# yabebalFantaye/MCEvidence

Hardware: AMD Instinct MI355X
Metric: knn_queries_per_sec (higher is better)
Workload: dtype f16 filter + f64 refine (exact f64 results)

## Files before the change

mcevidence_amd/csrc/f16_filter.hpp:

```cpp
#pragma once
#include <math.h>
#include <stdint.h>
#if defined(__HIPCC__)
#include <hip/hip_runtime.h>
#endif

#include "sym_types.hpp"

namespace mce {

#if defined(__HIPCC__)
#define MCE_HDI __host__ __device__ __forceinline__
#else
#define MCE_HDI inline
#endif

enum { HP_RMAX = 0, HP_SCALE = 1, HP_EY = 2, HP_YHATMAX = 3, HP_RHO = 4, HP_STAT_CHUNKS = 5, HP_STAT_TILES = 6, HP_COUNT = 16 };

constexpr int kHWaves = 8;
constexpr int kHThreads = kHWaves * 64;
constexpr int kHRelBits = 26;
constexpr int kHSymRowBits = kHRelBits - 1;

MCE_HDI float f16_round_up(double g)
{
#if defined(__HIP_DEVICE_COMPILE__)
    return __double2float_ru(g);
#else
    float f = (float)g;
    if ((double)f < g) f = nextafterf(f, __builtin_huge_valf());
    return f;
#endif
}
struct F16GateTerms { double a, c, eps; };
MCE_HDI double f16_gate_a(double ex, double ey, int KST) { return (ex + ey) * (1.0 + 1e-9) + 2.0 * sqrt(16.0 * KST) * 0x1p-14; }
MCE_HDI F16GateTerms f16_gate_terms(double ex, double xn, double ey, double ymax, double rho, int KST, bool live = true)
{
    const double r = sqrt(xn) + ymax;
    const double a = f16_gate_a(ex, ey, KST);
    const double eps = (32.0 * KST) * 0x1p-24 * r * r * (1.0 + 0x1p-9) + rho + 1e-30;
    return {a, live ? eps - xn : -__builtin_huge_val(), eps};
}
MCE_HDI double f16_reach2(double thr, double s2, double a)
{
    const double rr = sqrt(thr * s2) * (1.0 + 1e-12) + a;
    return rr * rr * (1.0 + 1e-12);
}
MCE_HDI float f16_gate_finite(double thr, double s2, double a, double c) { return f16_round_up(f16_reach2(thr, s2, a) + c); }
MCE_HDI float f16_gate(double thr, double s2, double a, double c)
{
    if (!(c > -__builtin_huge_val())) return -__builtin_huge_valf();
    if (!(thr < __builtin_huge_val())) return __builtin_huge_valf();
    return f16_gate_finite(thr, s2, a, c);
}
MCE_HDI double f16_row_const(double ymax) { return 0x1p-22 * (ymax * ymax + 1.0); }
MCE_HDI float f16_row_round(double g, double rowc) { return f16_round_up(g * (1.0 + 0x1p-22) + rowc + 1e-30); }
MCE_HDI float f16_row_gate(double thr, double s2, double a, double rowc)
{
    if (!(thr < __builtin_huge_val())) return __builtin_huge_valf();
    return f16_row_round(f16_reach2(thr, s2, a), rowc);
}
template <class P>
MCE_HDI float f16_row_gate_of(double thr, double ex, P params, int KST)
{
    if (!(thr < __builtin_huge_val())) return __builtin_huge_valf();
    const double s2 = params[HP_SCALE] * params[HP_SCALE];
    const double g = f16_reach2(thr, s2, f16_gate_a(ex, params[HP_EY], KST));
    return f16_row_round(g, f16_row_const(params[HP_YHATMAX]));
}
MCE_HDI double f16_seed_bound(double a_up, double xn, double eps, double a, double s2)
{
    const double dd = sqrt(fmax(a_up + xn + eps, 0.0)) * (1.0 + 1e-12) + a;
    return dd * dd * (1.0 + 1e-12) / s2 * (1.0 + 1e-12);
}

template <int N, class D, class I>
MCE_HD inline void list_insert(D&& own_d, I&& own_i, double d2, int j)
{
    const double INF = __builtin_huge_val();
    bool c_hi = (d2 < own_d[N - 1]) || (d2 == own_d[N - 1] && j < own_i[N - 1] && d2 < INF);
#pragma unroll
    for (int k = N - 1; k >= 1; --k) {
        const bool c_lo = (d2 < own_d[k - 1]) || (d2 == own_d[k - 1] && j < own_i[k - 1] && d2 < INF);
        own_d[k] = c_lo ? own_d[k - 1] : (c_hi ? d2 : own_d[k]);
        own_i[k] = c_lo ? own_i[k - 1] : (c_hi ? j : own_i[k]);
        c_hi = c_lo;
    }
    own_d[0] = c_hi ? d2 : own_d[0];
    own_i[0] = c_hi ? j : own_i[0];
}

#if defined(__HIPCC__)
typedef _Float16 v8h __attribute__((ext_vector_type(8)));
typedef float v16f __attribute__((ext_vector_type(16)));

__device__ __forceinline__ float min3f(float a, float b, float c)
{
    float r;
    asm("v_min3_f32 %0, %1, %2, %3" : "=v"(r) : "v"(a), "v"(b), "v"(c));
    return r;
}
__device__ __forceinline__ void f16_min16_halves(const v16f& c, float (&l1)[5], float& m0, float& m3)
{
    l1[0] = min3f(c[0], c[1], c[2]);
    l1[1] = min3f(c[3], c[4], c[5]);
    l1[2] = min3f(c[6], c[7], c[8]);
    l1[3] = min3f(c[9], c[10], c[11]);
    l1[4] = min3f(c[12], c[13], c[14]);
    m0 = min3f(l1[0], l1[1], l1[2]);
    m3 = min3f(l1[3], l1[4], c[15]);
}
__device__ __forceinline__ float f16_min16(const v16f& c, float (&l1)[5])
{
    float m0, m3;
    f16_min16_halves(c, l1, m0, m3);
    return min3f(m0, m3, m3);
}
__device__ __forceinline__ float f16_min16(const v16f& c, float (&l1)[5], float run)
{
    float m0, m3;
    f16_min16_halves(c, l1, m0, m3);
    return min3f(run, m0, m3);
}

template <int KCAP, class PS, class PT, class PR, class PF, class RG>
__device__ __forceinline__ bool sym_slot_insert(PS slots, PT thr, PR rrow, PF rtile, int ksel, int row, double d2, RG row_gate)
{
    const auto sl = slots + (int64_t)row * KCAP;
    for (;;) {
        double vmax = -1.0, v2 = -1.0;
        int imax = 0;
#pragma unroll
        for (int k = 0; k < KCAP; ++k) {
            if (k < ksel) {
                const double v = __longlong_as_double((long long)__hip_atomic_load(sl + k, __ATOMIC_RELAXED, __HIP_MEMORY_SCOPE_AGENT));
                if (v > vmax) { v2 = vmax; vmax = v; imax = k; }
                else if (v > v2) v2 = v;
            }
        }
        if (d2 > vmax) return false;
        if (d2 == vmax) return true;
        unsigned long long expect = (unsigned long long)__double_as_longlong(vmax);
        if (__hip_atomic_compare_exchange_strong(sl + imax, &expect, (unsigned long long)__double_as_longlong(d2), __ATOMIC_RELAXED,
                                                 __ATOMIC_RELAXED, __HIP_MEMORY_SCOPE_AGENT)) {
            const double nk = fmax(v2, d2);
            if (nk < __builtin_huge_val()) {
                const unsigned long long nb = (unsigned long long)__double_as_longlong(nk);
                const unsigned long long ob = __hip_atomic_fetch_min(thr + row, nb, __ATOMIC_RELAXED, __HIP_MEMORY_SCOPE_AGENT);
                if (nb < ob) {
                    const unsigned rb = __float_as_uint(row_gate(nk, row));
                    const unsigned orb = __hip_atomic_fetch_min(rrow + row, rb, __ATOMIC_RELAXED, __HIP_MEMORY_SCOPE_AGENT);
                    if (rb < orb) {
                        const auto rt = rrow + (int64_t)(row >> 5) * 32;
                        unsigned m = 0;
                        for (int k = 0; k < 32; ++k) {
                            const unsigned v = __hip_atomic_load(rt + k, __ATOMIC_RELAXED, __HIP_MEMORY_SCOPE_AGENT);
                            m = v > m ? v : m;
                        }
                        __hip_atomic_store(rtile + (row >> 5), __uint_as_float(m), __ATOMIC_RELAXED, __HIP_MEMORY_SCOPE_AGENT);
                    }
                }
            }
            return true;
        }
    }
}

template <bool ROWFLAG>
__device__ __forceinline__ unsigned f16_event(const v16f& c, const float (&l1)[5], const unsigned lanew, const float g, const bool rowflag, const int jb0,
                                              const unsigned todo, const int qlimit, int* const wq, int& qcount)
{
    const unsigned wbase = (lanew + (unsigned)jb0) | (ROWFLAG && rowflag ? (1u << kHSymRowBits) : 0u);
    unsigned rem = 0;
#define MCE_HIT(R_, P_, S_)                                                                                               \
    if ((S_) != 0 && (todo & (1u << (R_)))) {                                                                             \
        if (qcount > qlimit) rem |= 1u << (R_);                                                                           \
        else {                                                                                                            \
            if (P_) wq[__builtin_amdgcn_mbcnt_hi((unsigned)((S_) >> 32), __builtin_amdgcn_mbcnt_lo((unsigned)(S_), (unsigned)qcount))] = \
                        (int)(wbase + (unsigned)(((R_) & 3) + 8 * ((R_) >> 2)));                                          \
            qcount += __builtin_popcountll(S_);                                                                           \
        }                                                                                                                 \
    }
#define MCE_TRIPLE(I_, U_)                                                                                                \
    if ((U_) != 0) {                                                                                                      \
        const bool p0 = c[3 * (I_) + 0] <= g, p1 = c[3 * (I_) + 1] <= g, p2 = c[3 * (I_) + 2] <= g;                     \
        const unsigned long long s0 = __ballot(p0), s1 = __ballot(p1), s2 = __ballot(p2);                                \
        MCE_HIT(3 * (I_) + 0, p0, s0)                                                                                     \
        MCE_HIT(3 * (I_) + 1, p1, s1)                                                                                     \
        MCE_HIT(3 * (I_) + 2, p2, s2)                                                                                     \
    }
    const bool q0 = l1[0] <= g, q1 = l1[1] <= g, q2 = l1[2] <= g, q3 = l1[3] <= g, q4 = l1[4] <= g, p15 = c[15] <= g;
    const unsigned long long u0 = __ballot(q0), u1 = __ballot(q1), u2 = __ballot(q2), u3 = __ballot(q3), u4 = __ballot(q4), s15 = __ballot(p15);
    MCE_TRIPLE(0, u0) MCE_TRIPLE(1, u1) MCE_TRIPLE(2, u2) MCE_TRIPLE(3, u3) MCE_TRIPLE(4, u4)
    MCE_HIT(15, p15, s15)
#undef MCE_TRIPLE
#undef MCE_HIT
    return rem;
}

template <int VPT, class P>
__device__ __forceinline__ void f16_stage_chunk(P src, char* dst, int tid, int wave)
{
#pragma unroll
    for (int i = 0; i < VPT; ++i) {
        const int e = tid + i * kHThreads;
        __builtin_amdgcn_global_load_lds(
            (const __attribute__((address_space(1))) void*)(src + (size_t)e * 16),
            (__attribute__((address_space(3))) void*)(dst + (size_t)(wave * 64 + i * kHThreads) * 16),
            16, 0, 0);
    }
}
template <int KST>
__device__ __forceinline__ void f16_load_a(const char* lp, v8h (&a)[KST])
{
#pragma unroll
    for (int ks = 0; ks < KST; ++ks) a[ks] = *reinterpret_cast<const v8h*>(lp + ks * 1024);
}

#endif

}
```

mcevidence_amd/csrc/knn_panel.hpp:

```cpp
#pragma once
#include "knn_f16.hpp"

namespace mce {

struct PanelArgs {
    const _Float16* Yh;
    const _Float16* Xh;
    const double* qinfo;
    const double* params;
    const double* X;
    const double* Y;
    const int* rperm;
    double* part_d;
    int* part_i;
    int64_t nq, nr, nq_pad, self_offset;
    int D, ksel, self_exclude, spin_limit;
    int debug;
    SymParams sym;
    PanelGeom geom;
    const PanelUnit* units = nullptr;
    const double* lo_d = nullptr;
    const int* lo_i = nullptr;
};

#ifndef MCE_PANEL_STATS
#define MCE_PANEL_STATS 0
#endif
#ifndef MCE_PANEL_NPASS
#define MCE_PANEL_NPASS 3
#endif
#ifndef MCE_PANEL_STAGE_KB
#define MCE_PANEL_STAGE_KB MCE_H_STAGE_KB
#endif
#ifndef MCE_PANEL_QUEUE
#define MCE_PANEL_QUEUE MCE_H_QUEUE
#endif
#ifndef MCE_PANEL_TRIGGER
#define MCE_PANEL_TRIGGER 192
#endif
#ifndef MCE_PANEL_ABL
#define MCE_PANEL_ABL 0
#endif

__host__ __device__ constexpr int panel_chunk_tiles(int KST) { return MCE_PANEL_STAGE_KB / KST / 2 * 2; }
constexpr int kPanelQueue = MCE_PANEL_QUEUE;
__host__ __device__ constexpr size_t panel_lds_bytes(int KST)
{
    return (size_t)2 * panel_chunk_tiles(KST) * KST * 1024
           + (size_t)kHWaves * kPanelQueue * 16
           + (size_t)kHWaves * kHQT * 32 * 4 + 128
           + (size_t)kHWaves * kHQT * 32 * 4
           + (size_t)kHWaves * panel_chunk_tiles(KST) * kHQT * 4;
}

template <class T> __device__ __forceinline__ const __attribute__((address_space(1))) T* gptr(const T* p)
{
    return (const __attribute__((address_space(1))) T*)p;
}
template <class T> __device__ __forceinline__ __attribute__((address_space(1))) T* gptr_w(T* p)
{
    return (__attribute__((address_space(1))) T*)p;
}

__device__ __forceinline__ float vmaxf(float a, float b)
{
    float r;
    asm("v_max_f32 %0, %1, %2" : "=v"(r) : "v"(a), "v"(b));
    return r;
}

template <int KST, int KCAP, bool LOWER = false>
__global__ __launch_bounds__(kHThreads, 2) void knn_panel_kernel(PanelArgs args_by_value)
{
    static_assert(kHQT == 2 && kHNL == 1, "8 waves x 2 query tiles, one list per owner lane");
    constexpr int QT = 2;
    constexpr int QPW = 64;
    constexpr int QPB = kHWaves * QPW;
    constexpr int TPB = QPB / 32;
    constexpr int CT = panel_chunk_tiles(KST);
    constexpr int CHUNK_BYTES = CT * KST * 1024;
    constexpr int VPT = CHUNK_BYTES / 16 / kHThreads;
    static_assert(CHUNK_BYTES % (16 * kHThreads) == 0 && CT % 2 == 0, "chunk geometry");
    constexpr int QN = kPanelQueue;
    (void)args_by_value;
    typedef const __attribute__((address_space(4))) PanelArgs* ArgsPtr;
    const ArgsPtr ap0 = (ArgsPtr)__builtin_amdgcn_kernarg_segment_ptr();
#define MCE_ARGS() ([&]() __attribute__((always_inline)) { ArgsPtr p_ = ap0; asm volatile("" : "+s"(p_)); return p_; }())

    extern __shared__ __attribute__((aligned(16))) char lds_raw[];
    char* const stage0 = lds_raw;
    double* const qd2_all = reinterpret_cast<double*>(lds_raw + 2 * CHUNK_BYTES);
    int* const qpk_all = reinterpret_cast<int*>(qd2_all + kHWaves * QN);
    int* const qnx_all = qpk_all + kHWaves * QN;
    int* const head_all = qnx_all + kHWaves * QN;
    volatile int* const wvote = head_all + kHWaves * QPW;
    float* const sthr_all = reinterpret_cast<float*>(head_all + kHWaves * QPW + 32);
    int* const redo_all = reinterpret_cast<int*>(sthr_all + kHWaves * QPW);

    const int tid = threadIdx.x;
    const int lane = tid & 63;
    const int wave = __builtin_amdgcn_readfirstlane(tid >> 6);
    double* const wqd = qd2_all + wave * QN;
    int* const wq = qpk_all + wave * QN;
    int* const wnx = qnx_all + wave * QN;
    int* const whead = head_all + wave * QPW;
    float* const sthr = sthr_all + wave * QPW;
    int* const wredo = redo_all + wave * (CT * QT);
    const double INF = __builtin_huge_val();

#if MCE_PANEL_STATS
    const long long t_kernel0 = clock64();
    long long st_drains = 0, st_enq = 0, st_events = 0, st_redo = 0, st_tD = 0, st_tE = 0, st_tPro = 0, st_tA = 0, st_tR = 0, st_tB = 0;
#endif

    int sym_p, qblk, t_lo, t_hi, useq, sym_on, qb_lo;
    {
        const ArgsPtr a = MCE_ARGS();
        if (a->units) {
            const auto u = (const __attribute__((address_space(1))) PanelUnit*)a->units + blockIdx.x;
            qblk = __builtin_amdgcn_readfirstlane(u->qblk);
            t_lo = __builtin_amdgcn_readfirstlane(u->t_lo);
            t_hi = __builtin_amdgcn_readfirstlane(u->t_hi);
            useq = __builtin_amdgcn_readfirstlane(u->useq);
            sym_p = 0;
            sym_on = a->geom.sym_on;
            qb_lo = a->geom.qb_lo;
        } else {
            PanelGeom g;
            g.qb_lo = a->geom.qb_lo; g.qb_hi = a->geom.qb_hi; g.tpb = a->geom.tpb; g.tpp = a->geom.tpp;
            g.ct = a->geom.ct; g.ntiles = a->geom.ntiles; g.sym_on = a->geom.sym_on;
            panel_unit_decode((int)blockIdx.x, g, sym_p, qblk);
            panel_unit_tiles(sym_p, qblk, g, t_lo, t_hi);
            useq = panel_unit_seq(sym_p, qblk, g);
            sym_on = g.sym_on;
            qb_lo = g.qb_lo;
        }
    }
    auto chain_of = [&](int& chain, int64_t& list_off) __attribute__((always_inline)) {
        const ArgsPtr a = MCE_ARGS();
        chain = qblk;
        list_off = 0;
        if (a->units) {
            const auto u = (const __attribute__((address_space(1))) PanelUnit*)a->units + blockIdx.x;
            chain = __builtin_amdgcn_readfirstlane(u->chain);
            list_off = (int64_t)__builtin_amdgcn_readfirstlane(u->list_set) * KCAP * a->nq_pad;
        }
    };
    const int64_t qwave0 = (int64_t)qblk * QPB + wave * QPW;

    whead[lane] = -1;
    if (tid < 3) wvote[tid] = 0;

    double own_d[KCAP];
    int own_i[KCAP];
#pragma unroll
    for (int k = 0; k < KCAP; ++k) { own_d[k] = INF; own_i[k] = -1; }
    double seed_thr = INF;

    {
        const ArgsPtr a = MCE_ARGS();
        if (useq > 0) {
            int chain;
            int64_t list_off;
            chain_of(chain, list_off);
            int spins = 0;
            const int limit = ((a->debug & 16) && useq == 1 && (wave & 1)) ? -1 : a->spin_limit;
            bool ok = true;
            const auto done = gptr(a->sym.done);
            while (spins > limit || __hip_atomic_load(done + chain, __ATOMIC_RELAXED, __HIP_MEMORY_SCOPE_AGENT) < useq) {
                if (++spins > limit) { ok = false; break; }
                __builtin_amdgcn_s_sleep(32);
            }
            __builtin_amdgcn_fence(__ATOMIC_ACQUIRE, "agent");
            if (ok && gptr(a->sym.bucket_flag)[qblk] != 0) ok = false;
            if (ok) {
                const int64_t q = qwave0 + lane;
                const int64_t np = a->nq_pad;
                const auto pd = gptr(a->part_d) + list_off;
                const auto pi = gptr(a->part_i) + list_off;
#pragma unroll
                for (int k = 0; k < KCAP; ++k) {
                    own_d[k] = pd[(int64_t)k * np + q];
                    own_i[k] = pi[(int64_t)k * np + q];
                }
            } else if (lane == 0) {
                gptr_w(a->sym.bucket_flag)[qblk] = 1;
            }
        }
    }

    v8h b[QT][KST];
    float G[QT], cR[QT];
    unsigned lanew[QT];
    const int k_last = MCE_ARGS()->ksel - 1;
    {
        const ArgsPtr a = MCE_ARGS();
        const auto Xh = gptr(a->Xh);
#pragma unroll
        for (int qt = 0; qt < QT; ++qt) {
            const int64_t q = qwave0 + qt * 32 + (lane & 31);
#pragma unroll
            for (int ks = 0; ks < KST; ++ks)
                b[qt][ks] = *(const __attribute__((address_space(1))) v8h*)(Xh + q * (int64_t)(16 * KST) + 16 * ks + 8 * (lane >> 5));
            lanew[qt] = ((unsigned)(qt * 32 + (lane & 31)) << kHRelBits) | (unsigned)(4 * (lane >> 5));
            cR[qt] = -__builtin_huge_valf();
            G[qt] = -__builtin_huge_valf();
        }
    }
    double gq_a[QT], gq_c[QT], own_a = 0.0, s2c, rowc;
    {
        const ArgsPtr a = MCE_ARGS();
        const auto params = gptr(a->params);
        const auto qinfo = gptr(a->qinfo);
        const double p_scale = params[HP_SCALE], p_ey = params[HP_EY], p_ym = params[HP_YHATMAX], p_rho = params[HP_RHO];
        s2c = p_scale * p_scale;
        rowc = f16_row_const(p_ym);
#pragma unroll
        for (int qt = 0; qt < QT; ++qt) {
            const int64_t q = qwave0 + qt * 32 + (lane & 31);
            gq_a[qt] = 0.0;
            gq_c[qt] = -INF;
            if (q < a->nq && MCE_PANEL_ABL != 1) {
                const F16GateTerms t = f16_gate_terms(qinfo[2 * q], qinfo[2 * q + 1], p_ey, p_ym, p_rho, KST);
                gq_a[qt] = t.a;
                gq_c[qt] = t.c;
            }
        }
        {
            const int64_t q = qwave0 + lane;
            if (q < a->nq) own_a = f16_gate_a(qinfo[2 * q], p_ey, KST);
        }
    }
    auto gate_of = [&](double thr, int qt) __attribute__((always_inline)) -> float { return f16_gate(thr, s2c, gq_a[qt], gq_c[qt]); };
    auto own_row_gate = [&](double thr) __attribute__((always_inline)) -> float { return f16_row_gate(thr, s2c, own_a, rowc); };
    {
        const ArgsPtr a = MCE_ARGS();
        const int64_t q = qwave0 + lane;
        double t0 = INF;
        if (sym_on) t0 = __longlong_as_double((long long)__hip_atomic_load(gptr(a->sym.thr) + q, __ATOMIC_RELAXED, __HIP_MEMORY_SCOPE_AGENT));
        else if (a->sym.thr) t0 = __longlong_as_double((long long)gptr(a->sym.thr)[q]);
        seed_thr = t0;
        double tl = own_d[KCAP - 1];
#pragma unroll
        for (int k = 0; k < KCAP - 1; ++k) tl = (k == k_last) ? own_d[k] : tl;
        t0 = fmin(t0, tl);
        sthr[lane] = __double2float_ru(t0);
#pragma unroll
        for (int qt = 0; qt < QT; ++qt) G[qt] = gate_of(__shfl(t0, qt * 32 + (lane & 31), 64), qt);
        if (sym_on) {
#pragma unroll
            for (int qt = 0; qt < QT; ++qt) cR[qt] = gq_c[qt] > -INF ? f16_round_up(gq_c[qt]) : -__builtin_huge_valf();
        }
    }

    const int dbg_flags = MCE_ARGS()->debug;
    const int qlimit_gate = (dbg_flags & 8) ? -1 : QN - 64;
    int qcount = 0;
    int nredo = 0;

    auto drain = [&]() __attribute__((always_inline)) {
#if MCE_PANEL_STATS
        const long long t_d0 = clock64();
        st_drains += 1; st_enq += qcount;
#endif
        const ArgsPtr a = MCE_ARGS();
        const auto X = gptr(a->X);
        const auto Y = gptr(a->Y);
        const int D = a->D;
        const int64_t nq = a->nq, nr = a->nr;
        const int self_exclude = a->self_exclude;
        const int64_t self_offset = a->self_offset;
        const auto rperm = gptr(a->rperm);
        {
            const int sub = lane & 7;
            constexpr int NPASS = KST > 2 ? 1 : MCE_PANEL_NPASS;
            constexpr int EPL = KST > 2 ? 8 : 4;
            for (int b0 = 0; b0 < qcount; b0 += NPASS * 8) {
                int qlp[NPASS], ep[NPASS];
                bool okp[NPASS];
                const __attribute__((address_space(1))) double* xp[NPASS];
                const __attribute__((address_space(1))) double* yp[NPASS];
#pragma unroll
                for (int u = 0; u < NPASS; ++u) {
                    const int e = b0 + u * 8 + (lane >> 3);
                    ep[u] = e;
                    int ql = 0, j = 0;
                    const bool valid = e < qcount;
                    if (valid) {
                        const unsigned ent = (unsigned)wq[e];
                        ql = (int)(ent >> kHRelBits);
                        j = (int)(ent & ((1u << kHSymRowBits) - 1u));
                    }
                    qlp[u] = ql;
                    const int64_t q = qwave0 + ql;
                    okp[u] = valid && j < nr && q < nq && !(self_exclude && (int64_t)j == self_offset + q);
                    xp[u] = X + (okp[u] ? q : 0) * (int64_t)D;
                    yp[u] = Y + (okp[u] ? (int64_t)j : 0) * D;
                }
                double xv[NPASS][EPL], yv[NPASS][EPL];
#pragma unroll
                for (int u = 0; u < NPASS; ++u)
#pragma unroll
                    for (int v = 0; v < EPL; ++v) {
                        const int iv = (sub + 8 * v < D) ? sub + 8 * v : (sub < D ? sub : D - 1);
                        xv[u][v] = xp[u][iv];
                        yv[u][v] = yp[u][iv];
                    }
#pragma unroll
                for (int u = 0; u < NPASS; ++u) {
                    double a0 = 0.0;
#pragma unroll
                    for (int v = 0; v < EPL; ++v) {
                        const double t = (sub + 8 * v < D) ? xv[u][v] - yv[u][v] : 0.0;
                        a0 = fma(t, t, a0);
                    }
                    a0 += __shfl_xor(a0, 1, 64);
                    a0 += __shfl_xor(a0, 2, 64);
                    a0 += __shfl_xor(a0, 4, 64);
                    if (sub == 0 && ep[u] < qcount) {
                        wqd[ep[u]] = okp[u] ? a0 : -1.0;
                        bool col = okp[u] && !(a0 > (double)sthr[qlp[u]]);
                        if constexpr (LOWER) {
                            if (col) {
                                const int64_t o = (int64_t)(KCAP - 1) * a->nq_pad + qwave0 + qlp[u];
                                const double ld = gptr(a->lo_d)[o];
                                const int li = gptr(a->lo_i)[o];
                                const int jr = (int)((unsigned)wq[ep[u]] & ((1u << kHSymRowBits) - 1u));
                                const int jc = rperm ? rperm[jr] : jr;
                                col = a0 > ld || (a0 == ld && jc > li);
                            }
                        }
                        if (col) wnx[ep[u]] = atomicExch(&whead[qlp[u]], ep[u]);
                    }
                }
            }
        }
        __builtin_amdgcn_fence(__ATOMIC_ACQ_REL, "wavefront");
#if MCE_PANEL_STATS
        const long long t_dA = clock64();
        st_tA += t_dA - t_d0;
#endif
        {
            const auto sp_thr = gptr_w(a->sym.thr);
            const auto sp_rrow = gptr_w(a->sym.rrow);
            const auto sp_rtile = gptr_w(a->sym.rtile);
            const auto sp_slots = gptr_w(a->sym.slots);
            const auto sp_bucket_cnt = gptr_w(a->sym.bucket_cnt);
            const auto sp_bucket_flag = gptr_w(a->sym.bucket_flag);
            const auto sp_bucket = gptr_w(a->sym.bucket);
            const int sp_cap = a->sym.cap;
            const int ksel = a->ksel;
            auto row_gate = [&](double thr, int row) { return f16_row_gate_of(thr, gptr(a->qinfo)[2 * (int64_t)row], a->params, KST); };
            for (int e0 = 0; e0 < qcount; e0 += 64) {
                const int e = e0 + lane;
                const bool valid = e < qcount;
                const unsigned ent = valid ? (unsigned)wq[e] : 0u;
                const int ql = (int)(ent >> kHRelBits);
                const int j = (int)(ent & ((1u << kHSymRowBits) - 1u));
                const bool rowflag = (ent >> kHSymRowBits) & 1u;
                const double d2 = valid ? wqd[e] : -1.0;
                const bool ok = valid && d2 >= 0.0;
                const int oj = ok ? (rperm ? rperm[j] : j) : -1;
                bool rs = ok && rowflag;
                if (rs) {
                    const int jb = j / QPB;
                    rs = d2 <= __longlong_as_double((long long)__hip_atomic_load(sp_thr + j, __ATOMIC_RELAXED, __HIP_MEMORY_SCOPE_AGENT));
                    if constexpr (LOWER) {
                        if (rs) {
                            const int64_t o = (int64_t)(KCAP - 1) * a->nq_pad + j;
                            const double ld = gptr(a->lo_d)[o];
                            const int li = gptr(a->lo_i)[o];
                            const int sc = rperm ? rperm[qwave0 + ql] : (int)(qwave0 + ql);
                            rs = d2 > ld || (d2 == ld && sc > li);
                        }
                    }
                    if (rs) rs = sym_slot_insert<KCAP>(sp_slots, sp_thr, sp_rrow, sp_rtile, ksel, j, d2, row_gate);
                    if (rs) {
                        const int slot = __hip_atomic_fetch_add(sp_bucket_cnt + jb, 1, __ATOMIC_RELAXED, __HIP_MEMORY_SCOPE_AGENT);
                        if ((unsigned)slot < (unsigned)sp_cap) {
                            const auto en = sp_bucket + ((int64_t)jb * sp_cap + slot);
                            en->d2 = d2;
                            en->src = rperm ? rperm[qwave0 + ql] : (int)(qwave0 + ql);
                            en->row = j;
                        } else {
                            sp_bucket_flag[jb] = 1;
                        }
                    }
                }
                if (valid) wq[e] = oj;
            }
        }
        __builtin_amdgcn_fence(__ATOMIC_ACQ_REL, "wavefront");
#if MCE_PANEL_STATS
        const long long t_dR = clock64();
        st_tR += t_dR - t_dA;
#endif
        {
            int cur = whead[lane];
            whead[lane] = -1;
            while (__any(cur >= 0)) {
                const bool on = cur >= 0;
                const int ce = on ? cur : 0;
                const double d2 = on ? wqd[ce] : INF;
                const int j = wq[ce];
                cur = on ? wnx[ce] : -1;
                list_insert<KCAP>(own_d, own_i, d2, j);
            }
        }
        qcount = 0;
        double thr_own = own_d[KCAP - 1];
#pragma unroll
        for (int k = 0; k < KCAP - 1; ++k) thr_own = (k == k_last) ? own_d[k] : thr_own;
        thr_own = fmin(thr_own, seed_thr);
        if (sym_on) {
            const auto sp_thr = gptr_w(a->sym.thr);
            const auto sp_rrow = gptr_w(a->sym.rrow);
            const auto sp_rtile = gptr_w(a->sym.rtile);
            const int64_t q = qwave0 + lane;
            double t = thr_own;
            float R = 0.0f;
            if (q < nq) {
                if (t < INF) {
                    const unsigned long long mb = (unsigned long long)__double_as_longlong(t);
                    const unsigned rb = __float_as_uint(own_row_gate(t));
                    const unsigned long long ob = __hip_atomic_fetch_min(sp_thr + q, mb, __ATOMIC_RELAXED, __HIP_MEMORY_SCOPE_AGENT);
                    const unsigned orb = __hip_atomic_fetch_min(sp_rrow + q, rb, __ATOMIC_RELAXED, __HIP_MEMORY_SCOPE_AGENT);
                    t = fmin(t, __longlong_as_double((long long)ob));
                    R = __uint_as_float(rb < orb ? rb : orb);
                } else {
                    t = __longlong_as_double((long long)__hip_atomic_load(sp_thr + q, __ATOMIC_RELAXED, __HIP_MEMORY_SCOPE_AGENT));
                    const unsigned rb = __float_as_uint(own_row_gate(t));
                    const unsigned orb = __hip_atomic_fetch_min(sp_rrow + q, rb, __ATOMIC_RELAXED, __HIP_MEMORY_SCOPE_AGENT);
                    R = __uint_as_float(rb < orb ? rb : orb);
                }
            }
            thr_own = t;
            seed_thr = t;
            float m = R;
#pragma unroll
            for (int o = 16; o >= 1; o >>= 1) m = fmaxf(m, __shfl_xor(m, o, 64));
            if ((lane & 31) == 0) __hip_atomic_store(sp_rtile + ((qwave0 + lane) >> 5), m, __ATOMIC_RELAXED, __HIP_MEMORY_SCOPE_AGENT);
        }
        sthr[lane] = __double2float_ru(thr_own);
#pragma unroll
        for (int qt = 0; qt < QT; ++qt) G[qt] = gate_of(__shfl(thr_own, qt * 32 + (lane & 31), 64), qt);
#if MCE_PANEL_STATS
        st_tD += clock64() - t_d0;
#endif
    };

    auto event = [&](const v16f& c, const float (&l1)[5], const int qt, const float gq, const bool rowflag, const int jb0, const unsigned todo, const int qlimit) __attribute__((always_inline)) -> unsigned {
        return f16_event<true>(c, l1, lanew[qt], gq, rowflag, jb0, todo, qlimit, wq, qcount);
    };

    const auto Yh_bytes = (const __attribute__((address_space(1))) char*)MCE_ARGS()->Yh;
    auto stage_async = [&](int64_t c, int buf) { f16_stage_chunk<VPT>(Yh_bytes + c * (int64_t)CHUNK_BYTES, stage0 + buf * CHUNK_BYTES, tid, wave); };
    auto load_a = [&](const char* lp, v8h (&a)[KST]) { f16_load_a<KST>(lp, a); };
    auto mfma_first = [&](const v8h (&a)[KST], v16f (&acc)[QT]) __attribute__((always_inline)) {
#pragma unroll
        for (int qt = 0; qt < QT; ++qt) {
            v16f z = {0.f, 0.f, 0.f, 0.f, 0.f, 0.f, 0.f, 0.f, 0.f, 0.f, 0.f, 0.f, 0.f, 0.f, 0.f, 0.f};
            acc[qt] = __builtin_amdgcn_mfma_f32_32x32x16_f16(a[0], b[qt][0], z, 0, 0, 0);
        }
    };
    auto mfma_rest = [&](const v8h (&a)[KST], v16f (&acc)[QT]) __attribute__((always_inline)) {
#pragma unroll
        for (int ks = 1; ks < KST; ++ks)
#pragma unroll
            for (int qt = 0; qt < QT; ++qt) acc[qt] = __builtin_amdgcn_mfma_f32_32x32x16_f16(a[ks], b[qt][ks], acc[qt], 0, 0, 0);
    };
#if defined(__HIP_DEVICE_COMPILE__)
#define MCE_ORDER(GATED_, NEXT_) asm volatile("" : "+v"(GATED_[0]), "+v"(GATED_[1]), "+v"(NEXT_[0]), "+v"(NEXT_[1]))
#else
#define MCE_ORDER(GATED_, NEXT_) do {} while (0)
#endif
    auto gate_tile = [&](const v16f (&acc)[QT], const int jb0, const float (&gq)[QT], const float (&rg)[QT], const int tix) __attribute__((always_inline)) {
#if MCE_PANEL_ABL == 2
#if defined(__HIP_DEVICE_COMPILE__)
        asm volatile("" :: "v"(acc[0]), "v"(acc[1]));
#endif
        return;
#endif
        float l1[QT][5], mm[QT];
        bool pq[QT];
#pragma unroll
        for (int qt = 0; qt < QT; ++qt) {
            mm[qt] = f16_min16(acc[qt], l1[qt]);
            pq[qt] = mm[qt] <= gq[qt];
        }
        if (__any(pq[0] || pq[1])) {
#pragma unroll
            for (int qt = 0; qt < QT; ++qt) {
                if (!__any(pq[qt])) continue;
#if MCE_PANEL_STATS
                st_events += 1;
                const long long t_e0 = clock64();
#endif
                const unsigned rem = event(acc[qt], l1[qt], qt, gq[qt], mm[qt] <= rg[qt], jb0, 0xffffu, qlimit_gate);
                if (rem) {
                    if (lane == 0) wredo[nredo] = (int)(rem | ((unsigned)qt << 16) | ((unsigned)tix << 17));
                    nredo += 1;
                }
#if MCE_PANEL_STATS
                st_tE += clock64() - t_e0;
#endif
            }
        }
    };

    const int cfirst = t_lo / CT;
    const int ntot = (t_hi - 1) / CT - cfirst + 1;
    const auto rtile_p = gptr(MCE_ARGS()->sym.rtile);
    auto rt_load = [&](int c) -> float {
        const int t = c * CT + lane;
        const int tb = t / TPB;
        const bool en = sym_on && lane < CT && tb >= qb_lo && tb < qblk && MCE_PANEL_ABL != 1;
        const float r = en ? __hip_atomic_load(rtile_p + t, __ATOMIC_RELAXED, __HIP_MEMORY_SCOPE_AGENT) : -__builtin_huge_valf();
        return fmaxf(r, __shfl_xor(r, 1, 64));
    };
    float rt_cur = -__builtin_huge_valf(), rt_next;
    stage_async(cfirst, 0);
    rt_next = rt_load(cfirst);
#if MCE_PANEL_STATS
    st_tPro = clock64() - t_kernel0;
#endif
    v16f accA[QT], accB[QT];
    for (int k = 0; k < ntot; ++k) {
        const int buf = k & 1;
        const int c = cfirst + k;
        const int vs = k % 3;
        if (qcount >= MCE_PANEL_TRIGGER && lane == 0) wvote[vs] = 1;
#if MCE_PANEL_STATS
        const long long t_b0 = clock64();
#endif
        dma_barrier();
#if MCE_PANEL_STATS
        st_tB += clock64() - t_b0;
#endif
        if (tid == 0) wvote[vs == 0 ? 2 : vs - 1] = 0;
        rt_cur = rt_next;
        if (k + 1 < ntot) {
            stage_async(c + 1, buf ^ 1);
            rt_next = rt_load(c + 1);
        }
        bool need_drain = __builtin_amdgcn_readfirstlane(wvote[vs]) != 0 || k + 1 == ntot;
        const int tlo = (k == 0) ? t_lo - c * CT : 0;
        const int thi = t_hi - c * CT < CT ? t_hi - c * CT : CT;
        const char* const lbuf = stage0 + buf * CHUNK_BYTES + lane * 16;
        const int jchunk = c * (CT * 32);
        {
            v8h a0[KST], a1[KST];
            load_a(lbuf + (tlo * KST) * 1024, a0);
            load_a(lbuf + ((tlo + 1) * KST) * 1024, a1);
            mfma_first(a0, accA);
            mfma_rest(a0, accA);
            int t = tlo;
            float gqP[QT], rgP[QT];
            _Pragma("unroll 1") for (;;)
            {
                const float rP = __uint_as_float((unsigned)__builtin_amdgcn_readlane((int)__float_as_uint(rt_cur), t));
#pragma unroll
                for (int qt = 0; qt < QT; ++qt) {
                    rgP[qt] = rP + cR[qt];
                    gqP[qt] = vmaxf(G[qt], rgP[qt]);
                }
                const bool more = t + 2 < thi;
                load_a(lbuf + ((more ? t + 2 : t) * KST) * 1024, a0);
                mfma_first(a1, accB);
                MCE_ORDER(accA, accB);
                mfma_rest(a1, accB);
                gate_tile(accA, jchunk + t * 32, gqP, rgP, t);
                if (!more) break;
                load_a(lbuf + ((t + 3) * KST) * 1024, a1);
                mfma_first(a0, accA);
                MCE_ORDER(accB, accA);
                mfma_rest(a0, accA);
                gate_tile(accB, jchunk + (t + 1) * 32, gqP, rgP, t + 1);
                t += 2;
            }
            {
#if defined(__HIP_DEVICE_COMPILE__)
                asm volatile("s_nop 15\n\ts_nop 3" : "+v"(accB[0]), "+v"(accB[1]));
#endif
                gate_tile(accB, jchunk + (t + 1) * 32, gqP, rgP, t + 1);
            }
        }
        while (need_drain || nredo > 0 || (k + 1 == ntot && qcount > 0)) {
            drain();
            need_drain = false;
            const int n = nredo;
            nredo = 0;
            for (int i = 0; i < n; ++i) {
                const unsigned w = (unsigned)__builtin_amdgcn_readfirstlane(wredo[i]);
                const unsigned todo = w & 0xffffu;
                const int qt = (int)((w >> 16) & 1u), t = (int)(w >> 17);
                const float Rt = __uint_as_float((unsigned)__builtin_amdgcn_readlane((int)__float_as_uint(rt_cur), t));
                v8h at[KST];
                load_a(lbuf + (t * KST) * 1024, at);
                v16f z = {0.f, 0.f, 0.f, 0.f, 0.f, 0.f, 0.f, 0.f, 0.f, 0.f, 0.f, 0.f, 0.f, 0.f, 0.f, 0.f};
                v16f r_ = z;
                if (qt == 0) {
#pragma unroll
                    for (int ks = 0; ks < KST; ++ks) r_ = __builtin_amdgcn_mfma_f32_32x32x16_f16(at[ks], b[0][ks], r_, 0, 0, 0);
                } else {
#pragma unroll
                    for (int ks = 0; ks < KST; ++ks) r_ = __builtin_amdgcn_mfma_f32_32x32x16_f16(at[ks], b[1][ks], r_, 0, 0, 0);
                }
#if defined(__HIP_DEVICE_COMPILE__)
                asm volatile("s_nop 15\n\ts_nop 3" : "+v"(r_));
#endif
                float l1[5];
                const float mm = f16_min16(r_, l1);
                const float rg = Rt + (qt ? cR[1] : cR[0]);
                const float gq = vmaxf(qt ? G[1] : G[0], rg);
                unsigned rem = 0;
                if (__any(mm <= gq)) rem = event(r_, l1, qt, gq, mm <= rg, jchunk + t * 32, todo, QN - 64);
                if (rem) {
                    if (lane == 0) wredo[nredo] = (int)(rem | ((unsigned)qt << 16) | ((unsigned)t << 17));
                    nredo += 1;
                }
#if MCE_PANEL_STATS
                st_redo += 1;
#endif
            }
        }
    }

#if MCE_PANEL_STATS
    if (lane == 0) {
        const ArgsPtr a = MCE_ARGS();
        double* o = const_cast<double*>(a->params) + 16 + ((int64_t)blockIdx.x * kHWaves + wave) * 8;
        o[0] = (double)st_drains; o[1] = (double)st_enq; o[2] = (double)st_redo; o[3] = (double)st_events;
        o[4] = (double)st_tE; o[5] = (double)st_tD; o[6] = (double)(clock64() - t_kernel0); o[7] = (double)st_tPro;
        double* o2 = const_cast<double*>(a->params) + 16 + ((int64_t)gridDim.x * kHWaves) * 8 + ((int64_t)blockIdx.x * kHWaves + wave) * 8;
        o2[0] = (double)st_tA; o2[1] = (double)st_tR; o2[2] = (double)(st_tD - st_tA - st_tR); o2[3] = (double)st_tB; o2[4] = 0; o2[5] = 0; o2[6] = 0; o2[7] = 0;
    }
#endif
    {
        const ArgsPtr a = MCE_ARGS();
        const int64_t q = qwave0 + lane;
        const int64_t np = a->nq_pad;
        int chain;
        int64_t list_off;
        chain_of(chain, list_off);
        const auto pd = gptr_w(a->part_d) + list_off;
        const auto pi = gptr_w(a->part_i) + list_off;
#pragma unroll
        for (int k = 0; k < KCAP; ++k) {
            pd[(int64_t)k * np + q] = own_d[k];
            pi[(int64_t)k * np + q] = own_i[k];
        }
        __builtin_amdgcn_fence(__ATOMIC_RELEASE, "agent");
        __syncthreads();
        if (tid == 0) __hip_atomic_fetch_add(gptr_w(a->sym.done) + chain, 1, __ATOMIC_RELAXED, __HIP_MEMORY_SCOPE_AGENT);
    }
#undef MCE_ARGS
}

}
```

Baseline: 26.36 million.

## Defer gate hits to a software-pipelined recompute loop after each chunk

The in-loop gate no longer resolves candidate hits inline. It only records which tiles and query halves fired into a per-wave list. After the chunk, a new loop recomputes those tiles with MFMA, double-buffering the LDS A-fragment loads and MFMAs of the next entry while the current one is settled, and a flat 16-ballot resolve replaces the hierarchical event routine. This aims to keep the main MFMA loop free of divergent enqueue work, at the cost of recomputing every fired tile and more register pressure.

```diff
diff --git a/mcevidence_amd/csrc/f16_filter.hpp b/mcevidence_amd/csrc/f16_filter.hpp
--- a/mcevidence_amd/csrc/f16_filter.hpp
+++ b/mcevidence_amd/csrc/f16_filter.hpp
@@ -198,6 +198,30 @@
     return rem;
 }
 
+template <bool ROWFLAG>
+__device__ __forceinline__ unsigned f16_resolve(const v16f& c, const unsigned lanew, const float g, const bool rowflag, const int jb0, const unsigned todo,
+                                                const int qlimit, int* const wq, int& qcount)
+{
+    const unsigned wbase = (lanew + (unsigned)jb0) | (ROWFLAG && rowflag ? (1u << kHSymRowBits) : 0u);
+    unsigned long long s[16];
+#pragma unroll
+    for (int r = 0; r < 16; ++r) s[r] = __ballot(c[r] <= g);
+    unsigned rem = 0;
+#pragma unroll
+    for (int r = 0; r < 16; ++r) {
+        if (s[r] != 0 && (todo & (1u << r))) {
+            if (qcount > qlimit) rem |= 1u << r;
+            else {
+                if (c[r] <= g)
+                    wq[__builtin_amdgcn_mbcnt_hi((unsigned)(s[r] >> 32), __builtin_amdgcn_mbcnt_lo((unsigned)s[r], (unsigned)qcount))] =
+                        (int)(wbase + (unsigned)((r & 3) + 8 * (r >> 2)));
+                qcount += __builtin_popcountll(s[r]);
+            }
+        }
+    }
+    return rem;
+}
+
 template <int VPT, class P>
 __device__ __forceinline__ void f16_stage_chunk(P src, char* dst, int tid, int wave)
 {
diff --git a/mcevidence_amd/csrc/knn_panel.hpp b/mcevidence_amd/csrc/knn_panel.hpp
--- a/mcevidence_amd/csrc/knn_panel.hpp
+++ b/mcevidence_amd/csrc/knn_panel.hpp
@@ -110,7 +110,7 @@
 
 #if MCE_PANEL_STATS
     const long long t_kernel0 = clock64();
-    long long st_drains = 0, st_enq = 0, st_events = 0, st_redo = 0, st_tD = 0, st_tE = 0, st_tPro = 0, st_tA = 0, st_tR = 0, st_tB = 0;
+    long long st_drains = 0, st_enq = 0, st_events = 0, st_redo = 0, st_tD = 0, st_tE = 0, st_tPro = 0, st_tA = 0, st_tR = 0, st_tB = 0, st_tL = 0;
 #endif
 
     int sym_p, qblk, t_lo, t_hi, useq, sym_on, qb_lo;
@@ -254,7 +254,7 @@
     }
 
     const int dbg_flags = MCE_ARGS()->debug;
-    const int qlimit_gate = (dbg_flags & 8) ? -1 : QN - 64;
+    const bool dbg_drain_each = (dbg_flags & 8) != 0;
     int qcount = 0;
     int nredo = 0;
 
@@ -449,9 +449,6 @@
 #endif
     };
 
-    auto event = [&](const v16f& c, const float (&l1)[5], const int qt, const float gq, const bool rowflag, const int jb0, const unsigned todo, const int qlimit) __attribute__((always_inline)) -> unsigned {
-        return f16_event<true>(c, l1, lanew[qt], gq, rowflag, jb0, todo, qlimit, wq, qcount);
-    };
 
     const auto Yh_bytes = (const __attribute__((address_space(1))) char*)MCE_ARGS()->Yh;
     auto stage_async = [&](int64_t c, int buf) { f16_stage_chunk<VPT>(Yh_bytes + c * (int64_t)CHUNK_BYTES, stage0 + buf * CHUNK_BYTES, tid, wave); };
@@ -474,7 +471,7 @@
 #else
 #define MCE_ORDER(GATED_, NEXT_) do {} while (0)
 #endif
-    auto gate_tile = [&](const v16f (&acc)[QT], const int jb0, const float (&gq)[QT], const float (&rg)[QT], const int tix) __attribute__((always_inline)) {
+    auto gate_tile = [&](const v16f (&acc)[QT], const float (&gq)[QT], const int tix) __attribute__((always_inline)) {
 #if MCE_PANEL_ABL == 2
 #if defined(__HIP_DEVICE_COMPILE__)
         asm volatile("" :: "v"(acc[0]), "v"(acc[1]));
@@ -488,22 +485,16 @@
             mm[qt] = f16_min16(acc[qt], l1[qt]);
             pq[qt] = mm[qt] <= gq[qt];
         }
-        if (__any(pq[0] || pq[1])) {
-#pragma unroll
-            for (int qt = 0; qt < QT; ++qt) {
-                if (!__any(pq[qt])) continue;
-#if MCE_PANEL_STATS
-                st_events += 1;
-                const long long t_e0 = clock64();
-#endif
-                const unsigned rem = event(acc[qt], l1[qt], qt, gq[qt], mm[qt] <= rg[qt], jb0, 0xffffu, qlimit_gate);
-                if (rem) {
-                    if (lane == 0) wredo[nredo] = (int)(rem | ((unsigned)qt << 16) | ((unsigned)tix << 17));
-                    nredo += 1;
-                }
-#if MCE_PANEL_STATS
-                st_tE += clock64() - t_e0;
-#endif
+        const unsigned long long m0 = __ballot(pq[0]), m1 = __ballot(pq[1]);
+        if ((m0 | m1) != 0) {
+            const unsigned w0 = 0xffffu | ((unsigned)tix << 17);
+            if (m0 != 0) {
+                if (lane == 0) wredo[nredo] = (int)w0;
+                nredo += 1;
+            }
+            if (m1 != 0) {
+                if (lane == 0) wredo[nredo] = (int)(w0 | (1u << 16));
+                nredo += 1;
             }
         }
     };
@@ -555,74 +546,158 @@
             mfma_first(a0, accA);
             mfma_rest(a0, accA);
             int t = tlo;
-            float gqP[QT], rgP[QT];
+            float gqP[QT];
             _Pragma("unroll 1") for (;;)
             {
                 const float rP = __uint_as_float((unsigned)__builtin_amdgcn_readlane((int)__float_as_uint(rt_cur), t));
 #pragma unroll
                 for (int qt = 0; qt < QT; ++qt) {
-                    rgP[qt] = rP + cR[qt];
-                    gqP[qt] = vmaxf(G[qt], rgP[qt]);
+                    gqP[qt] = vmaxf(G[qt], rP + cR[qt]);
                 }
                 const bool more = t + 2 < thi;
                 load_a(lbuf + ((more ? t + 2 : t) * KST) * 1024, a0);
                 mfma_first(a1, accB);
                 MCE_ORDER(accA, accB);
                 mfma_rest(a1, accB);
-                gate_tile(accA, jchunk + t * 32, gqP, rgP, t);
+                gate_tile(accA, gqP, t);
                 if (!more) break;
                 load_a(lbuf + ((t + 3) * KST) * 1024, a1);
                 mfma_first(a0, accA);
                 MCE_ORDER(accB, accA);
                 mfma_rest(a0, accA);
-                gate_tile(accB, jchunk + (t + 1) * 32, gqP, rgP, t + 1);
+                gate_tile(accB, gqP, t + 1);
                 t += 2;
             }
             {
 #if defined(__HIP_DEVICE_COMPILE__)
                 asm volatile("s_nop 15\n\ts_nop 3" : "+v"(accB[0]), "+v"(accB[1]));
 #endif
-                gate_tile(accB, jchunk + (t + 1) * 32, gqP, rgP, t + 1);
-            }
-        }
-        while (need_drain || nredo > 0 || (k + 1 == ntot && qcount > 0)) {
-            drain();
-            need_drain = false;
+                gate_tile(accB, gqP, t + 1);
+            }
+        }
+        {
             const int n = nredo;
             nredo = 0;
-            for (int i = 0; i < n; ++i) {
-                const unsigned w = (unsigned)__builtin_amdgcn_readfirstlane(wredo[i]);
-                const unsigned todo = w & 0xffffu;
+#if MCE_PANEL_STATS
+            const long long t_l0 = clock64(), t_lD = st_tD;
+#endif
+            constexpr int NW = (CT * QT + 63) / 64;
+            int wv[NW];
+#pragma unroll
+            for (int u = 0; u < NW; ++u) wv[u] = (u * 64 + lane < CT * QT) ? wredo[u * 64 + lane] : 0;
+            auto word = [&](const int i) __attribute__((always_inline)) -> unsigned {
+                int w = __builtin_amdgcn_readlane(wv[0], i & 63);
+#pragma unroll
+                for (int u = 1; u < NW; ++u) w = (i >> 6) == u ? __builtin_amdgcn_readlane(wv[u], i & 63) : w;
+                return (unsigned)w;
+            };
+            auto fetch = [&](const unsigned w, v8h (&at)[KST]) __attribute__((always_inline)) { load_a(lbuf + ((int)(w >> 17) * KST) * 1024, at); };
+            auto mult = [&](const unsigned w, const v8h (&at)[KST], v16f& r) __attribute__((always_inline)) {
+                const v16f z = {0.f, 0.f, 0.f, 0.f, 0.f, 0.f, 0.f, 0.f, 0.f, 0.f, 0.f, 0.f, 0.f, 0.f, 0.f, 0.f};
+                if (((w >> 16) & 1u) == 0) {
+                    r = __builtin_amdgcn_mfma_f32_32x32x16_f16(at[0], b[0][0], z, 0, 0, 0);
+#pragma unroll
+                    for (int ks = 1; ks < KST; ++ks) r = __builtin_amdgcn_mfma_f32_32x32x16_f16(at[ks], b[0][ks], r, 0, 0, 0);
+                } else {
+                    r = __builtin_amdgcn_mfma_f32_32x32x16_f16(at[0], b[1][0], z, 0, 0, 0);
+#pragma unroll
+                    for (int ks = 1; ks < KST; ++ks) r = __builtin_amdgcn_mfma_f32_32x32x16_f16(at[ks], b[1][ks], r, 0, 0, 0);
+                }
+            };
+            auto settle = [&](const unsigned w, const unsigned todo, const v16f& r, bool& fired) __attribute__((always_inline)) -> unsigned {
                 const int qt = (int)((w >> 16) & 1u), t = (int)(w >> 17);
                 const float Rt = __uint_as_float((unsigned)__builtin_amdgcn_readlane((int)__float_as_uint(rt_cur), t));
-                v8h at[KST];
-                load_a(lbuf + (t * KST) * 1024, at);
-                v16f z = {0.f, 0.f, 0.f, 0.f, 0.f, 0.f, 0.f, 0.f, 0.f, 0.f, 0.f, 0.f, 0.f, 0.f, 0.f, 0.f};
-                v16f r_ = z;
-                if (qt == 0) {
-#pragma unroll
-                    for (int ks = 0; ks < KST; ++ks) r_ = __builtin_amdgcn_mfma_f32_32x32x16_f16(at[ks], b[0][ks], r_, 0, 0, 0);
-                } else {
-#pragma unroll
-                    for (int ks = 0; ks < KST; ++ks) r_ = __builtin_amdgcn_mfma_f32_32x32x16_f16(at[ks], b[1][ks], r_, 0, 0, 0);
-                }
+                float l1[5];
+                const float mm = f16_min16(r, l1);
+                float c0 = cR[0], c1 = cR[1], g0 = G[0], g1 = G[1];
 #if defined(__HIP_DEVICE_COMPILE__)
-                asm volatile("s_nop 15\n\ts_nop 3" : "+v"(r_));
-#endif
-                float l1[5];
-                const float mm = f16_min16(r_, l1);
-                const float rg = Rt + (qt ? cR[1] : cR[0]);
-                const float gq = vmaxf(qt ? G[1] : G[0], rg);
+                asm("" : "+v"(c0), "+v"(c1), "+v"(g0), "+v"(g1));
+#endif
+                const float rg = Rt + (qt ? c1 : c0);
+                const float gq = vmaxf(qt ? g1 : g0, rg);
                 unsigned rem = 0;
-                if (__any(mm <= gq)) rem = event(r_, l1, qt, gq, mm <= rg, jchunk + t * 32, todo, QN - 64);
-                if (rem) {
-                    if (lane == 0) wredo[nredo] = (int)(rem | ((unsigned)qt << 16) | ((unsigned)t << 17));
-                    nredo += 1;
+                fired = __any(mm <= gq);
+                if (fired) {
+#if MCE_PANEL_STATS
+                    st_events += 1;
+                    const long long t_e0 = clock64();
+#endif
+                    rem = f16_resolve<true>(r, lanew[0] + ((unsigned)qt << (kHRelBits + 5)), gq, mm <= rg, jchunk + t * 32, todo, QN - 64, wq, qcount);
+                    rem = (unsigned)__builtin_amdgcn_readfirstlane((int)rem);
+                    qcount = __builtin_amdgcn_readfirstlane(qcount);
+#if MCE_PANEL_STATS
+                    st_tE += clock64() - t_e0;
+#endif
                 }
 #if MCE_PANEL_STATS
                 st_redo += 1;
 #endif
-            }
+                return rem;
+            };
+            int i = 0;
+            unsigned todo = 0xffffu;
+            for (;;) {
+                bool full = false;
+                if (i < n) {
+                    v16f r[2];
+                    v8h at[2][KST];
+#if defined(__HIP_DEVICE_COMPILE__)
+                    asm volatile("" : "=v"(r[1]));
+#pragma unroll
+                    for (int ks = 0; ks < KST; ++ks) asm volatile("" : "=v"(at[1][ks]));
+#endif
+                    unsigned wcur = word(i), wnext = 0, wnn = 0;
+                    fetch(wcur, at[0]);
+                    mult(wcur, at[0], r[0]);
+                    if (i + 1 < n) {
+                        wnext = word(i + 1);
+                        fetch(wnext, at[1]);
+                    }
+                    auto step = [&](v16f& rc, v8h (&ac)[KST], v16f& rn, v8h (&an)[KST]) __attribute__((always_inline)) -> bool {
+                        if (i + 1 < n) {
+                            mult(wnext, an, rn);
+                            if (i + 2 < n) {
+                                wnn = word(i + 2);
+                                fetch(wnn, ac);
+                            }
+#if defined(__HIP_DEVICE_COMPILE__)
+                            if constexpr (KST >= 2) asm volatile("" : "+v"(rc), "+v"(rn));
+                            else asm volatile("s_nop 3" : "+v"(rc), "+v"(rn));
+#endif
+                        } else {
+#if defined(__HIP_DEVICE_COMPILE__)
+                            asm volatile("s_nop 15\n\ts_nop 3" : "+v"(rc));
+#endif
+                        }
+                        bool fired;
+                        const unsigned rem = settle(wcur, todo, rc, fired);
+                        if (rem != 0 || (fired && dbg_drain_each)) {
+                            todo = rem;
+                            full = true;
+                            return true;
+                        }
+                        i += 1;
+                        todo = 0xffffu;
+                        wcur = wnext;
+                        wnext = wnn;
+                        return i >= n;
+                    };
+                    for (;;) {
+                        if (step(r[0], at[0], r[1], at[1])) break;
+                        if (step(r[1], at[1], r[0], at[0])) break;
+                    }
+                }
+                if (!(full || need_drain)) break;
+                drain();
+                if (!full) break;
+                if (todo == 0) {
+                    i += 1;
+                    todo = 0xffffu;
+                }
+            }
+#if MCE_PANEL_STATS
+            st_tL += clock64() - t_l0 - (st_tD - t_lD);
+#endif
         }
     }
 
@@ -633,7 +708,7 @@
         o[0] = (double)st_drains; o[1] = (double)st_enq; o[2] = (double)st_redo; o[3] = (double)st_events;
         o[4] = (double)st_tE; o[5] = (double)st_tD; o[6] = (double)(clock64() - t_kernel0); o[7] = (double)st_tPro;
         double* o2 = const_cast<double*>(a->params) + 16 + ((int64_t)gridDim.x * kHWaves) * 8 + ((int64_t)blockIdx.x * kHWaves + wave) * 8;
-        o2[0] = (double)st_tA; o2[1] = (double)st_tR; o2[2] = (double)(st_tD - st_tA - st_tR); o2[3] = (double)st_tB; o2[4] = 0; o2[5] = 0; o2[6] = 0; o2[7] = 0;
+        o2[0] = (double)st_tA; o2[1] = (double)st_tR; o2[2] = (double)(st_tD - st_tA - st_tR); o2[3] = (double)st_tB; o2[4] = (double)st_tL; o2[5] = 0; o2[6] = 0; o2[7] = 0;
     }
 #endif
     {
```

New measurement: 19.68 million. 0.747x the previous value.
